# NVlabs/FB-BEV

Hardware: AMD Instinct MI355X
Metric: multi-cam samples/sec (forward view transformation: lift + voxel ranking + bev_pool_v2) (higher is better)
Workload: dtype f32

## Files before the change

fb_bev_amd/csrc/capi.hip:

```cpp
#include <stdio.h>
#include <stdlib.h>
#include <mutex>
#include "rt.h"
#include "pool_kernels.h"
#include "pool_bwd_kernels.h"
#include "rank_kernels.h"
#include "sort_kernels.h"
#include "msda_kernels.h"
#include "geom_kernels.h"
#include "da_kernels.h"
#include "history_kernels.h"
#include "norm_kernels.h"
#include "history_conv_kernels.h"
#include "history_fused_kernels.h"
#include "history_conv_x3_kernels.h"
#include "history_fused_x3_kernels.h"
#include "rows_linear_kernels.h"
#include "rows_linear_f32_kernels.h"
#include "da_fused_kernels.h"
#include "da_bwd_planes_kernels.h"
#include "msda_bwd_kernels.h"
#include "conv3d_kernels.h"
#include "det_kernels.h"
#include "occ_kernels.h"
#include "../../include/fbbev.h"

#include "capi_common.h"

extern "C" int fbbev_version(void) { return 100; }

extern "C" int fbbev_bev_pool_v2_fwd(int c, int n_intervals, const float* depth, const float* feat,
                                     const int32_t* ranks_depth, const int32_t* ranks_feat,
                                     const int32_t* ranks_bev, const int32_t* interval_starts,
                                     const int32_t* interval_lengths, float* out,
                                     fbbev_stream_t stream_) {
    if (c <= 0 || n_intervals < 0) return FBBEV_E_BADARG;
    if (n_intervals == 0) return 0;
    if (!depth || !feat || !ranks_depth || !ranks_feat || !ranks_bev || !interval_starts ||
        !interval_lengths || !out) return FBBEV_E_BADARG;
    fbbev_rt_stream stream = (fbbev_rt_stream)stream_;
    if (c % 4 == 0 && aligned16(feat) && aligned16(out)) {
        const long long threads = (long long)n_intervals * (c / 4);
        FBBEV_LAUNCH(k_pool_fwd_rows<4>, (threads + 255) / 256, 256, 0, stream, c, n_intervals, depth,
                     feat, ranks_depth, ranks_feat, ranks_bev, interval_starts, interval_lengths, out);
    } else {
        const long long threads = (long long)n_intervals * c;
        FBBEV_LAUNCH(k_pool_fwd_rows<1>, (threads + 255) / 256, 256, 0, stream, c, n_intervals, depth,
                     feat, ranks_depth, ranks_feat, ranks_bev, interval_starts, interval_lengths, out);
    }
    FBBEV_CHECK_LAUNCH();
    return 0;
}

extern "C" int fbbev_bev_pool_v2_bwd(int c, int n_intervals, const float* out_grad,
                                     const float* depth, const float* feat,
                                     const int32_t* ranks_depth, const int32_t* ranks_feat,
                                     const int32_t* ranks_bev, const int32_t* interval_starts,
                                     const int32_t* interval_lengths, float* depth_grad,
                                     float* feat_grad, fbbev_stream_t stream_) {
    if (c <= 0 || n_intervals < 0) return FBBEV_E_BADARG;
    if (c > 256) return FBBEV_E_UNSUPPORTED;
    if (n_intervals == 0) return 0;
    if (!out_grad || !depth || !feat || !ranks_depth || !ranks_feat || !ranks_bev ||
        !interval_starts || !interval_lengths || !depth_grad || !feat_grad) return FBBEV_E_BADARG;
    fbbev_rt_stream stream = (fbbev_rt_stream)stream_;
    const long long blocks = ((long long)n_intervals * 64 + 255) / 256;
    const int nch = (c + 63) / 64;
#define FBBEV_BWD(NCH)                                                                             \
    FBBEV_LAUNCH(k_pool_bwd<NCH>, blocks, 256, 0, stream, c, n_intervals, out_grad, depth, feat,   \
                 ranks_depth, ranks_feat, ranks_bev, interval_starts, interval_lengths, depth_grad, \
                 feat_grad)
    switch (nch) {
        case 1: FBBEV_BWD(1); break;
        case 2: FBBEV_BWD(2); break;
        case 3: FBBEV_BWD(3); break;
        default: FBBEV_BWD(4); break;
    }
#undef FBBEV_BWD
    FBBEV_CHECK_LAUNCH();
    return 0;
}

extern "C" int fbbev_lidar_coor(const float* xs, const float* ys, const float* ds, const float* rots,
                                const float* trans, const float* intrins, const float* post_rots,
                                const float* post_trans, const float* bda, int B, int N, int D, int H,
                                int W, float* coor, fbbev_stream_t stream_) {
    if (B <= 0 || N <= 0 || D <= 0 || H <= 0 || W <= 0) return FBBEV_E_BADARG;
    if (!xs || !ys || !ds || !rots || !trans || !intrins || !post_rots || !post_trans || !bda || !coor)
        return FBBEV_E_BADARG;
    const long long dhw = (long long)D * H * W;
    const long long chunks = (dhw + 255) / 256;
    if (chunks * B * N >= (1ll << 31)) return FBBEV_E_UNSUPPORTED;
    fbbev_cam_ptrs g;
    g.xs = xs; g.ys = ys; g.ds = ds; g.rots = rots; g.trans = trans; g.intrins = intrins; g.post_rots = post_rots;
    g.post_trans = post_trans; g.bda = bda; g.N = N; g.D = D; g.H = H; g.W = W;
    FBBEV_LAUNCH(k_lidar_coor, chunks * B * N, 256, 0, (fbbev_rt_stream)stream_, g, (int)chunks, coor);
    FBBEV_CHECK_LAUNCH();
    return 0;
}

extern "C" int fbbev_nchw_to_nhwc(const float* in, float* out, int n_images, int C, int HW, fbbev_stream_t stream_) {
    return fbbev_tokens_from_nchw(in, out, n_images, C, HW, (long long)C * HW, 0, nullptr, 0, stream_);
}

static int tokens_from_nchw_impl(const float* in, float* out, int n_images, int C, int HW, long long out_image_stride,
                                 long long out_offset, const float* bias, int bias_rows, const float* pos_bias,
                                 fbbev_stream_t stream_) {
    if (n_images < 0 || C <= 0 || HW <= 0 || out_offset < 0 || out_image_stride < (long long)C * HW) return FBBEV_E_BADARG;
    if (bias && bias_rows <= 0) return FBBEV_E_BADARG;
    if (n_images == 0) return 0;
    if (!in || !out) return FBBEV_E_BADARG;
    const int tc = (C + 31) / 32, th = (HW + 31) / 32;
    const long long blocks = (long long)n_images * tc * th;
    if (blocks >= (1ll << 31)) return FBBEV_E_UNSUPPORTED;
    FBBEV_LAUNCH(k_nchw_to_nhwc, blocks, 256, 0, (fbbev_rt_stream)stream_, in, out, C, HW, tc, th, out_image_stride,
                 out_offset, bias, bias ? bias_rows : 1, pos_bias);
    FBBEV_CHECK_LAUNCH();
    return 0;
}

extern "C" int fbbev_tokens_from_nchw(const float* in, float* out, int n_images, int C, int HW,
                                      long long out_image_stride, long long out_offset, const float* bias,
                                      int bias_rows, fbbev_stream_t stream_) {
    return tokens_from_nchw_impl(in, out, n_images, C, HW, out_image_stride, out_offset, bias, bias_rows, nullptr, stream_);
}

extern "C" int fbbev_tokens_from_nchw_levels(const float* const* in, const int32_t* hw, int n_levels, float* out, int n_images, int C,
                                             const float* bias, int bias_rows, fbbev_stream_t stream_) {
    if (n_levels <= 0 || n_levels > 8 || n_images < 0 || C <= 0 || !in || !hw) return FBBEV_E_BADARG;
    if (bias && bias_rows <= 0) return FBBEV_E_BADARG;
    if (n_images == 0) return 0;
    if (!out) return FBBEV_E_BADARG;
    fbbev_token_levels lv;
    const int tc = (C + 31) / 32;
    long long start = 0, blocks = 0;
    for (int l = 0; l < 8; ++l) { lv.in[l] = nullptr; lv.out_off[l] = 0; lv.hw[l] = 1; lv.blk0[l] = 0; }
    for (int l = 0; l < n_levels; ++l) {
        if (hw[l] <= 0 || !in[l]) return FBBEV_E_BADARG;
        lv.in[l] = in[l]; lv.hw[l] = hw[l]; lv.out_off[l] = start * C; lv.blk0[l] = (int)blocks;
        start += hw[l];
        blocks += (long long)n_images * tc * ((hw[l] + 31) / 32);
        if (blocks >= (1ll << 31)) return FBBEV_E_UNSUPPORTED;
    }
    lv.blk0[n_levels] = (int)blocks;
    lv.n = n_levels;
    FBBEV_LAUNCH(k_nchw_to_nhwc_levels, blocks, 256, 0, (fbbev_rt_stream)stream_, lv, out, C, tc, start * C, bias, bias ? bias_rows : 1);
    FBBEV_CHECK_LAUNCH();
    return 0;
}

extern "C" int fbbev_tokens_from_nchw_pos(const float* in, float* out, int n_images, int C, int HW, long long out_image_stride,
                                          long long out_offset, const float* pos_bias, fbbev_stream_t stream_) {
    if (!pos_bias) return FBBEV_E_BADARG;
    return tokens_from_nchw_impl(in, out, n_images, C, HW, out_image_stride, out_offset, nullptr, 0, pos_bias, stream_);
}

extern "C" int fbbev_point_sampling(const float* xs, const float* ys, const float* zs, const float* rots,
                                    const float* trans, const float* intrins, const float* post_rots,
                                    const float* post_trans, const float* bda, int B, int N, int Y, int X,
                                    int Za, float ogfH, float ogfW, float* ref_cam, uint8_t* mask,
                                    float* qdepth, fbbev_stream_t stream_) {
    if (B <= 0 || N <= 0 || Y <= 0 || X <= 0 || Za <= 0 || !(ogfH > 0.f) || !(ogfW > 0.f)) return FBBEV_E_BADARG;
    if (!xs || !ys || !zs || !rots || !trans || !intrins || !post_rots || !post_trans || !bda || !ref_cam ||
        !mask || !qdepth) return FBBEV_E_BADARG;
    const long long npts = (long long)Y * X * Za;
    int ppt = 8;
    while (ppt > 1 && (npts + 256 * ppt - 1) / (256 * ppt) * B * N < 1024) ppt >>= 1;
    const long long chunks = (npts + 256 * ppt - 1) / (256 * ppt);
    if (chunks * B * N >= (1ll << 31) || ((uintptr_t)ref_cam & 7) != 0) return FBBEV_E_UNSUPPORTED;
    FBBEV_LAUNCH(k_point_sampling, chunks * B * N, 256, 0, (fbbev_rt_stream)stream_, xs, ys, zs, rots, trans,
                 intrins, post_rots, post_trans, bda, B, N, Y, X, Za, ogfH, ogfW, (int)chunks, ref_cam, mask,
                 qdepth, ppt);
    FBBEV_CHECK_LAUNCH();
    return 0;
}

static inline int key_bits(long long total_voxels) {
    int bits = 1;
    while ((1ll << bits) < total_voxels) ++bits;
    return bits;
}

static const int kSortTile[7] = {2048, 4096, 8192, 12288, 16384, 4096, 8192};
static int sort_variant_for(long long items) {
    for (int v = 0; v < 5; ++v)
        if ((items + kSortTile[v] - 1) / kSortTile[v] <= 256) return v;
    return 6;
}
static const int kIvTile[3] = {1024, 4096, 8192};
static int iv_variant_for(long long items) {
    for (int v = 0; v < 3; ++v)
        if ((items + kIvTile[v] - 1) / kIvTile[v] <= 256) return v;
    return 2;
}

static fbbev_fastdiv make_fastdiv(unsigned int d) {
    fbbev_fastdiv f;
    f.d = d; f.m = 0; f.sh = 0;
    if (d <= 1) { f.d = 1; return f; }
    unsigned int l = 0;
    while ((1ull << l) < d) ++l;
    f.m = (unsigned int)((((1ull << l) - d) << 32) / d + 1);
    f.sh = l - 1;
    return f;
}

struct rank_ws_layout {
    size_t keys_a, keys_t, vals_t, matrix, ctot, chunk_info, total;
    int v0, wgs0;
    int v1, wgs1;
    int vi, wgsi;
};

static rank_ws_layout rank_layout(long long n) {
    rank_ws_layout L;
    L.v0 = sort_variant_for(n);
    L.v1 = sort_variant_for((n + 1) / 2);
    L.vi = iv_variant_for((n + 1) / 2);
    if (const char* env = fbbev_env_str("FBBEV_RANK_SHAPE")) {
        int a = -1, b = -1, c = -1;
        if (sscanf(env, "%d,%d,%d", &a, &b, &c) == 3 && a >= 0 && a < 7 && b >= 0 && b < 7 && c >= 0 && c < 3) {
            L.v0 = a; L.v1 = b; L.vi = c;
        }
    }
    L.wgs0 = (int)((n + kSortTile[L.v0] - 1) / kSortTile[L.v0]);
    L.wgs1 = (int)((n + kSortTile[L.v1] - 1) / kSortTile[L.v1]);
    L.wgsi = (int)((n + kIvTile[L.vi] - 1) / kIvTile[L.vi]);
    size_t off = 0;
    L.keys_a = off; off = align_up(off + (size_t)n * 4, 256);
    L.keys_t = off; off = align_up(off + (size_t)n * 4, 256);
    L.vals_t = off; off = align_up(off + (size_t)n * 4, 256);
    const int rows = L.wgs0 > L.wgs1 ? L.wgs0 : L.wgs1;
    const size_t seg_rows = (size_t)(n / FBBEV_SEG_TILE) + 256 + 1;
    size_t mbytes = (size_t)rows * FBBEV_SORT_MAX_NB * 4;
    if (seg_rows * FBBEV_SEG_NB * 4 > mbytes) mbytes = seg_rows * FBBEV_SEG_NB * 4;
    L.matrix = off; off = align_up(off + mbytes, 256);
    L.ctot = off; off = align_up(off + seg_rows * 4, 256);
    L.chunk_info = off; off = align_up(off + (size_t)L.wgsi * 8, 256);
    L.total = off;
    return L;
}

#define FBBEV_SORT_DISPATCH(KERNEL, v, by_waves, grid, stream, ...)                                             \
    do {                                                                                                        \
        switch (v) {                                                                                            \
            case 0: FBBEV_LAUNCH((KERNEL<(by_waves) ? 4 : 256, 8>), grid, 256, 0, stream, __VA_ARGS__); break;   \
            case 1: FBBEV_LAUNCH((KERNEL<(by_waves) ? 16 : 1024, 4>), grid, 1024, 0, stream, __VA_ARGS__); break; \
            case 2: FBBEV_LAUNCH((KERNEL<(by_waves) ? 16 : 1024, 8>), grid, 1024, 0, stream, __VA_ARGS__); break; \
            case 3: FBBEV_LAUNCH((KERNEL<(by_waves) ? 16 : 1024, 12>), grid, 1024, 0, stream, __VA_ARGS__); break; \
            case 5: FBBEV_LAUNCH((KERNEL<(by_waves) ? 8 : 512, 8>), grid, 512, 0, stream, __VA_ARGS__); break;     \
            case 6: FBBEV_LAUNCH((KERNEL<(by_waves) ? 8 : 512, 16>), grid, 512, 0, stream, __VA_ARGS__); break;    \
            default: FBBEV_LAUNCH((KERNEL<(by_waves) ? 16 : 1024, 16>), grid, 1024, 0, stream, __VA_ARGS__); break; \
        }                                                                                                       \
    } while (0)

extern "C" size_t fbbev_rank_workspace_bytes(int64_t n_points) {
    if (n_points <= 0) return 256;
    return rank_layout(n_points).total;
}

static int rank_seg_mode() { FBBEV_KNOB_ONCE(int, m, fbbev_env_int("FBBEV_RANK_SEG", -1)); return m; }

static int rank_build_impl(const float* coor, const fbbev_cam_ptrs* cams, const float* frustum, int B, int N, int D,
                           int H, int W,
                           const float* lower3, const float* interval3, const float* grid_size3,
                           int32_t* ranks_bev, int32_t* ranks_depth, int32_t* ranks_feat,
                           int32_t* interval_starts, int32_t* interval_lengths, int32_t* interval_rank,
                           int32_t* counts, void* workspace, size_t workspace_bytes, fbbev_rt_stream stream,
                           const float* point_depth = nullptr, float depth_thr = 0.f, const int* skip = nullptr) {
    if (B <= 0 || N <= 0 || D <= 0 || H <= 0 || W <= 0) return FBBEV_E_BADARG;
    if (point_depth && cams) return FBBEV_E_UNSUPPORTED;
    if ((!coor && !cams) || !lower3 || !interval3 || !grid_size3 || !ranks_bev || !ranks_depth || !ranks_feat ||
        !interval_starts || !interval_lengths || !counts || !workspace) return FBBEV_E_BADARG;
    const long long n = (long long)B * N * D * H * W;
    if (n >= (1ll << 30)) return FBBEV_E_UNSUPPORTED;
    const rank_ws_layout L = rank_layout(n);
    if (workspace_bytes < L.total) return FBBEV_E_WORKSPACE;
    unsigned char* ws = static_cast<unsigned char*>(workspace);
    unsigned int* keys_a = reinterpret_cast<unsigned int*>(ws + L.keys_a);
    unsigned int* keys_t = reinterpret_cast<unsigned int*>(ws + L.keys_t);
    unsigned int* vals_t = reinterpret_cast<unsigned int*>(ws + L.vals_t);
    int* matrix = reinterpret_cast<int*>(ws + L.matrix);
    int2* chunk_info = reinterpret_cast<int2*>(ws + L.chunk_info);

    fbbev_grid_params gp;
    gp.lx = lower3[0]; gp.ly = lower3[1]; gp.lz = lower3[2];
    gp.ix = interval3[0]; gp.iy = interval3[1]; gp.iz = interval3[2];
    gp.gx = grid_size3[0]; gp.gy = grid_size3[1]; gp.gz = grid_size3[2];
    volatile float zy = gp.gz * gp.gy;
    volatile float zyx = zy * gp.gx;
    volatile float yx = gp.gy * gp.gx;
    gp.f_zyx = zyx; gp.f_yx = yx;
    const long long total_voxels = (long long)B * (long long)gp.gz * (long long)gp.gy * (long long)gp.gx;
    if (total_voxels <= 0 || total_voxels >= (1ll << 30)) return FBBEV_E_UNSUPPORTED;
    const int bits = key_bits(total_voxels + 128);
    struct { int passes, rb; } plan;
    plan.passes = (bits + FBBEV_SORT_MAX_RB - 1) / FBBEV_SORT_MAX_RB;
    plan.rb = (bits + plan.passes - 1) / plan.passes;
    if (plan.rb < 4) plan.rb = 4;
    const int rb = plan.rb;
    const int seg_mode = rank_seg_mode();
    const long long vps = total_voxels / B;
    const long long npb = n / B;
    const int lbits = key_bits(vps);
    const bool seg_legal = B <= 256 && total_voxels <= (1ll << 24) && lbits <= 2 * FBBEV_SEG_RB;
    const long long seg_cps = (npb + FBBEV_SEG_TILE - 1) / FBBEV_SEG_TILE;
    const bool seg = seg_legal && seg_mode != 0 &&
                     (seg_mode == 2 || ((lbits + FBBEV_SEG_RB - 1) / FBBEV_SEG_RB < plan.passes && seg_cps <= 64 && B * seg_cps >= 96));
    if (seg) {
        fbbev_seg sg;
        sg.npb = (int)npb; sg.cps = (int)((npb + FBBEV_SEG_TILE - 1) / FBBEV_SEG_TILE); sg.vps = (unsigned int)vps; sg.nseg = B;
        const int passes = (lbits + FBBEV_SEG_RB - 1) / FBBEV_SEG_RB;
        const int srb = (lbits + passes - 1) / passes < 4 ? 4 : (lbits + passes - 1) / passes;
        const int wgs = B * sg.cps;
        int* ctot = reinterpret_cast<int*>(ws + L.ctot);
        fbbev_geom_src gs;
        if (cams) { gs.cam = *cams; gs.frustum = frustum; gs.gp = gp; }
        else { gs.cam = fbbev_cam_ptrs(); gs.frustum = nullptr; gs.gp = gp; }
        if (cams) FBBEV_LAUNCH((k_keys_hist_seg<true>), wgs, FBBEV_SEG_NT, 0, stream, gs, (const float*)nullptr, gp, (const float*)nullptr, 0.f,
                               sg, srb, skip, keys_a, matrix, ctot);
        else FBBEV_LAUNCH((k_keys_hist_seg<false>), wgs, FBBEV_SEG_NT, 0, stream, gs, coor, gp, point_depth, depth_thr, sg, srb, skip, keys_a,
                          matrix, ctot);
        FBBEV_CHECK_LAUNCH();
        const unsigned int* kin = keys_a;
        const unsigned int* vin = nullptr;
        static const int pairs = fbbev_env_int("FBBEV_RANK_PAIRS", 1);
        for (int p = 0; p < passes; ++p) {
            const bool to_out = p == passes - 1;
            const int pm = pairs ? ((p > 0 ? 1 : 0) | (to_out ? 0 : 2)) : 0;
            unsigned int* ko = to_out ? reinterpret_cast<unsigned int*>(ranks_bev) : keys_t;
            unsigned int* vo = to_out ? reinterpret_cast<unsigned int*>(ranks_depth) : vals_t;
            if (p > 0) {
                FBBEV_LAUNCH(k_sort_hist_seg, wgs, FBBEV_SEG_NT, 0, stream, kin, (const int*)ctot, sg, p * srb, srb, skip, matrix,
                             (pm & 1) ? 2 : 1);
                FBBEV_CHECK_LAUNCH();
            }
            static const int swz = fbbev_env_int("FBBEV_RANK_XCD_SWIZZLE", 1);
            const int sw = (swz && B >= 8) ? 1 : 0;
            FBBEV_LAUNCH(k_sort_scatter_seg, sw ? (wgs + 7) / 8 * 8 : wgs, FBBEV_SEG_NT, 0, stream, kin, vin, (const int*)matrix,
                         (const int*)ctot, sg, p, srb, skip, ko, vo, counts, sw, pm);
            FBBEV_CHECK_LAUNCH();
            kin = ko; vin = vo;
        }
    } else {
    if (cams) {
            fbbev_geom_src gs;
            gs.cam = *cams; gs.frustum = frustum; gs.gp = gp;
            FBBEV_SORT_DISPATCH(k_keys_hist_geom, L.v0, false, L.wgs0, stream, gs, n, rb, skip, keys_a, matrix);
        } else {
            FBBEV_SORT_DISPATCH(k_keys_hist_coor, L.v0, false, L.wgs0, stream, coor, n, n / B, gp, point_depth, depth_thr, rb, keys_a, matrix);
        }
        FBBEV_CHECK_LAUNCH();
        const unsigned int* kin = keys_a;
        const unsigned int* vin = nullptr;
        for (int p = 0; p < plan.passes; ++p) {
            const bool to_out = ((plan.passes - 1 - p) % 2) == 0;
            unsigned int* ko = to_out ? reinterpret_cast<unsigned int*>(ranks_bev) : keys_t;
            unsigned int* vo = to_out ? reinterpret_cast<unsigned int*>(ranks_depth) : vals_t;
            const int v = p == 0 ? L.v0 : L.v1, wgs = p == 0 ? L.wgs0 : L.wgs1;
            if (p > 0) {
                FBBEV_SORT_DISPATCH(k_sort_hist, v, false, wgs, stream, kin, (const int*)counts, p * rb, rb, skip, matrix);
                FBBEV_CHECK_LAUNCH();
            }
            static const int swz = fbbev_env_int("FBBEV_RANK_XCD_SWIZZLE", 1);
            const bool sw = swz == 2 && p == 0;
            FBBEV_SORT_DISPATCH(k_sort_scatter, v, true, sw ? (wgs + 7) / 8 * 8 : wgs, stream, kin, vin, n, (const int*)matrix, p, rb, skip,
                                ko, vo, counts, sw ? wgs : 0);
            FBBEV_CHECK_LAUNCH();
            kin = ko; vin = vo;
        }
}
    const unsigned int* keys = reinterpret_cast<const unsigned int*>(ranks_bev);
    const unsigned int* vals = reinterpret_cast<const unsigned int*>(ranks_depth);
    const fbbev_fastdiv div_dhw = make_fastdiv((unsigned int)((long long)D * H * W)), div_hw = make_fastdiv((unsigned int)(H * W));
    switch (L.vi) {
        case 0:
            FBBEV_LAUNCH((k_interval_count<4, 4>), L.wgsi, 256, 0, stream, keys, (const int*)counts, skip, chunk_info);
            FBBEV_LAUNCH((k_interval_write<4, 4>), L.wgsi, 256, (size_t)2 * 4 * 256 * 4, stream, keys, vals, div_dhw, div_hw, (const int2*)chunk_info, skip,
                         ranks_feat, interval_starts, interval_lengths, interval_rank, counts);
            break;
        case 1:
            FBBEV_LAUNCH((k_interval_count<16, 4>), L.wgsi, 1024, 0, stream, keys, (const int*)counts, skip, chunk_info);
            FBBEV_LAUNCH((k_interval_write<16, 4>), L.wgsi, 1024, (size_t)2 * 4 * 1024 * 4, stream, keys, vals, div_dhw, div_hw, (const int2*)chunk_info, skip,
                         ranks_feat, interval_starts, interval_lengths, interval_rank, counts);
            break;
        default:
            FBBEV_LAUNCH((k_interval_count<16, 8>), L.wgsi, 1024, 0, stream, keys, (const int*)counts, skip, chunk_info);
            FBBEV_LAUNCH((k_interval_write<16, 8>), L.wgsi, 1024, (size_t)2 * 8 * 1024 * 4, stream, keys, vals, div_dhw, div_hw, (const int2*)chunk_info, skip,
                         ranks_feat, interval_starts, interval_lengths, interval_rank, counts);
            break;
    }
    FBBEV_CHECK_LAUNCH();
    return 0;
}

extern "C" int fbbev_rank_build(const float* coor, int B, int N, int D, int H, int W,
                                const float* lower3, const float* interval3,
                                const float* grid_size3, int32_t* ranks_bev, int32_t* ranks_depth,
                                int32_t* ranks_feat, int32_t* interval_starts,
                                int32_t* interval_lengths, int32_t* interval_rank, int32_t* counts,
                                void* workspace, size_t workspace_bytes, fbbev_stream_t stream_) {
    if (!coor) return FBBEV_E_BADARG;
    return rank_build_impl(coor, nullptr, nullptr, B, N, D, H, W, lower3, interval3, grid_size3, ranks_bev, ranks_depth,
                           ranks_feat, interval_starts, interval_lengths, interval_rank, counts, workspace,
                           workspace_bytes, (fbbev_rt_stream)stream_);
}

extern "C" int fbbev_rank_build_depth(const float* coor, const float* depth, float depth_threshold, int B, int N, int D,
                                      int H, int W, const float* lower3, const float* interval3,
                                      const float* grid_size3, int32_t* ranks_bev, int32_t* ranks_depth,
                                      int32_t* ranks_feat, int32_t* interval_starts, int32_t* interval_lengths,
                                      int32_t* interval_rank, int32_t* counts, void* workspace, size_t workspace_bytes,
                                      fbbev_stream_t stream_) {
    if (!coor || !depth) return FBBEV_E_BADARG;
    return rank_build_impl(coor, nullptr, nullptr, B, N, D, H, W, lower3, interval3, grid_size3, ranks_bev, ranks_depth,
                           ranks_feat, interval_starts, interval_lengths, interval_rank, counts, workspace,
                           workspace_bytes, (fbbev_rt_stream)stream_, depth, depth_threshold);
}

static int lift_rank_build_impl(const float* frustum, const float* xs, const float* ys, const float* ds,
                                const float* rots, const float* trans, const float* intrins, const float* post_rots,
                                const float* post_trans, const float* bda, int B, int N, int D, int H, int W,
                                const float* lower3, const float* interval3, const float* grid_size3,
                                int32_t* ranks_bev, int32_t* ranks_depth, int32_t* ranks_feat, int32_t* interval_starts,
                                int32_t* interval_lengths, int32_t* interval_rank, int32_t* counts, void* workspace,
                                size_t workspace_bytes, fbbev_rt_stream stream, uint32_t* cam_key, int32_t* cache_state) {
    if (!xs || !ys || !ds || !rots || !trans || !intrins || !post_rots || !post_trans || !bda) return FBBEV_E_BADARG;
    if (B <= 0 || N <= 0) return FBBEV_E_BADARG;
    fbbev_cam_ptrs g;
    g.xs = xs; g.ys = ys; g.ds = ds; g.rots = rots; g.trans = trans; g.intrins = intrins; g.post_rots = post_rots;
    g.post_trans = post_trans; g.bda = bda; g.N = N; g.D = D; g.H = H; g.W = W;
    const int* skip = nullptr;
    if (cam_key) {
        if (!cache_state) return FBBEV_E_BADARG;
        FBBEV_LAUNCH(k_cam_key, 1, 256, 0, stream, g, B, cam_key, cache_state);
        FBBEV_CHECK_LAUNCH();
        skip = cache_state;
    }
    return rank_build_impl(nullptr, &g, frustum, B, N, D, H, W, lower3, interval3, grid_size3, ranks_bev, ranks_depth,
                           ranks_feat, interval_starts, interval_lengths, interval_rank, counts, workspace,
                           workspace_bytes, stream, nullptr, 0.f, skip);
}

extern "C" int fbbev_lift_rank_build(const float* frustum, const float* xs, const float* ys, const float* ds,
                                     const float* rots,
                                     const float* trans, const float* intrins, const float* post_rots,
                                     const float* post_trans, const float* bda, int B, int N, int D, int H,
                                     int W, const float* lower3, const float* interval3,
                                     const float* grid_size3, int32_t* ranks_bev, int32_t* ranks_depth,
                                     int32_t* ranks_feat, int32_t* interval_starts, int32_t* interval_lengths,
                                     int32_t* interval_rank, int32_t* counts, void* workspace,
                                     size_t workspace_bytes, fbbev_stream_t stream_) {
    return lift_rank_build_impl(frustum, xs, ys, ds, rots, trans, intrins, post_rots, post_trans, bda, B, N, D, H, W, lower3,
                                interval3, grid_size3, ranks_bev, ranks_depth, ranks_feat, interval_starts,
                                interval_lengths, interval_rank, counts, workspace, workspace_bytes,
                                (fbbev_rt_stream)stream_, nullptr, nullptr);
}

extern "C" size_t fbbev_cam_key_words(int B, int N) {
    return (B <= 0 || N <= 0) ? 0 : (size_t)B * N * 33 + (size_t)B * 9;
}

extern "C" int fbbev_lift_rank_build_cached(const float* frustum, const float* xs, const float* ys, const float* ds,
                                            const float* rots, const float* trans, const float* intrins,
                                            const float* post_rots, const float* post_trans, const float* bda, int B,
                                            int N, int D, int H, int W, const float* lower3, const float* interval3,
                                            const float* grid_size3, int32_t* ranks_bev, int32_t* ranks_depth,
                                            int32_t* ranks_feat, int32_t* interval_starts, int32_t* interval_lengths,
                                            int32_t* interval_rank, int32_t* counts, void* workspace,
                                            size_t workspace_bytes, uint32_t* cam_key, int32_t* cache_state,
                                            fbbev_stream_t stream_) {
    if (!cam_key || !cache_state) return FBBEV_E_BADARG;
    return lift_rank_build_impl(frustum, xs, ys, ds, rots, trans, intrins, post_rots, post_trans, bda, B, N, D, H, W, lower3,
                                interval3, grid_size3, ranks_bev, ranks_depth, ranks_feat, interval_starts,
                                interval_lengths, interval_rank, counts, workspace, workspace_bytes,
                                (fbbev_rt_stream)stream_, cam_key, cache_state);
}

static inline int pick_tile(int tile_voxels) {
    switch (tile_voxels) { case 64: case 128: case 256: case 512: case 1024: return tile_voxels; default: return 64; }
}
static inline int small_tile_shift(int tile_voxels) {
    switch (tile_voxels) { case 8: return 3; case 16: return 4; case 32: return 5; default: return 0; }
}

extern "C" size_t fbbev_pool_dense_workspace_bytes(int B, int Z, int Y, int X) {
    if (B <= 0 || Z <= 0 || Y <= 0 || X <= 0) return 256;
    const long long yx = (long long)Y * X;
    const long long tiles = ((long long)B * Z * yx + 7) / 8 + (long long)B * Z;
    return align_up((size_t)(tiles + 2) * 8, 256);
}

static int pool_tile_index_impl(const int32_t* interval_rank, const int32_t* interval_starts,
// ... 3173 lines not shown
```

fb_bev_amd/csrc/sort_kernels.h:

```cpp
#pragma once
#include "rt.h"
#include "geom_kernels.h"
#include "rank_kernels.h"

#define FBBEV_SORT_MAX_RB 8
#define FBBEV_SORT_MAX_NB (1 << FBBEV_SORT_MAX_RB)
#define FBBEV_SORT_MAX_PASSES 4
#define FBBEV_DROP_KEY 0xffffffffu

__device__ __forceinline__ bool fbbev_skip(const int* skip) { return skip != nullptr && *skip != 0; }

struct fbbev_geom_src {
    fbbev_cam_ptrs cam;
    const float* frustum;
    fbbev_grid_params gp;
};

__device__ __forceinline__ unsigned int fbbev_geom_key(const fbbev_geom_src& g, const float* m, int cam, int i) {
    float u, v, dep;
    if (g.frustum) {
        u = g.frustum[3 * i]; v = g.frustum[3 * i + 1]; dep = g.frustum[3 * i + 2];
    } else {
        const int w = i % g.cam.W, h = (i / g.cam.W) % g.cam.H, d = i / (g.cam.W * g.cam.H);
        u = g.cam.xs[w]; v = g.cam.ys[h]; dep = g.cam.ds[d];
// ... 67 lines not shown
            if (key != FBBEV_DROP_KEY) atomicAdd(&cnt[key & dmask], 1);
        }
    }
    __syncthreads();
    for (int d = threadIdx.x; d < nb; d += NT) matrix[(long long)blockIdx.x * nb + d] = cnt[d];
}

template <int NT, int PER>
__global__ void __launch_bounds__(NT)
k_sort_hist(const unsigned int* __restrict__ keys, const int* __restrict__ counts, int shift, int rb,
            const int* __restrict__ skip, int* __restrict__ matrix) {
    if (fbbev_skip(skip)) return;
    __shared__ int cnt[FBBEV_SORT_MAX_NB];
    const int nb = 1 << rb;
    const unsigned int dmask = (unsigned int)nb - 1u;
    const long long n = counts[0];
    const long long base = (long long)blockIdx.x * (NT * PER);
    if (base >= n) return;
    for (int d = threadIdx.x; d < nb; d += NT) cnt[d] = 0;
    __syncthreads();
    unsigned int key[PER];
#pragma unroll
    for (int r = 0; r < PER; ++r) {
        const long long idx = base + threadIdx.x + r * NT;
        key[r] = (idx < n) ? keys[idx] : FBBEV_DROP_KEY;
    }
#pragma unroll
    for (int r = 0; r < PER; ++r)
        if (key[r] != FBBEV_DROP_KEY) atomicAdd(&cnt[(key[r] >> shift) & dmask], 1);
    __syncthreads();
    for (int d = threadIdx.x; d < nb; d += NT) matrix[(long long)blockIdx.x * nb + d] = cnt[d];
}

template <int WAVES, int ROUNDS>
__global__ void __launch_bounds__(WAVES * 64)
k_sort_scatter(const unsigned int* __restrict__ keys_in, const unsigned int* __restrict__ vals_in, long long n_host,
               const int* __restrict__ matrix, int pass, int rb, const int* __restrict__ skip,
               unsigned int* __restrict__ keys_out, unsigned int* __restrict__ vals_out, int* __restrict__ counts, int swz_chunks) {
    if (fbbev_skip(skip)) return;
    constexpr int NT = WAVES * 64;
    constexpr int TILE = NT * ROUNDS;
    constexpr int NBM = FBBEV_SORT_MAX_NB;
    __shared__ int cnt[WAVES][NBM];
    __shared__ int woff[WAVES][NBM];
    __shared__ int pos0[NBM];
    __shared__ int ldsw[WAVES];
    const int tid = threadIdx.x, wave = tid >> 6, lane = tid & 63;
    const int nb = 1 << rb, shift = pass * rb;
    const unsigned int dmask = (unsigned int)nb - 1u;
    int wg = (int)blockIdx.x;
    if (swz_chunks > 0) {
        wg = (int)(blockIdx.x & 7) * ((swz_chunks + 7) >> 3) + (int)(blockIdx.x >> 3);
        if (wg >= swz_chunks) return;
    }
    const long long n = (pass == 0) ? n_host : (long long)counts[0];
    const long long chunk0 = (long long)wg * TILE;
    if (chunk0 >= n) {
        if (pass == 0 && n_host <= 0 && wg == 0 && tid == 0) counts[0] = 0;
        return;
    }
    for (int i = tid; i < WAVES * NBM; i += NT) (&cnt[0][0])[i] = 0;
    const int rows = (int)((n + TILE - 1) / TILE);
    {
        const int groups = NT / nb > 0 ? NT / nb : 1;
        int pre = 0, all = 0;
        if (tid < groups * nb) {
            const int d = tid % nb, rg = tid / nb;
            constexpr int U = 8;
            int r = rg;
            for (; r + (U - 1) * groups < rows; r += U * groups) {
                int c[U];
#pragma unroll
                for (int u = 0; u < U; ++u) c[u] = matrix[(long long)(r + u * groups) * nb + d];
#pragma unroll
                for (int u = 0; u < U; ++u) { all += c[u]; if (r + u * groups < wg) pre += c[u]; }
            }
            for (; r < rows; r += groups) {
                const int c = matrix[(long long)r * nb + d];
                all += c;
                if (r < wg) pre += c;
            }
        }
        int* red = &woff[0][0];
        __syncthreads();
        if (tid < groups * nb) { red[tid] = pre; red[groups * nb + tid] = all; }
        __syncthreads();
        int mypre = 0, myall = 0;
        if (tid < nb) {
            for (int gi = 0; gi < groups; ++gi) { mypre += red[gi * nb + tid]; myall += red[groups * nb + gi * nb + tid]; }
        }
        __syncthreads();
        int total;
        const int dbase = fbbev_block_excl_scan_w<WAVES, false>(tid < nb ? myall : 0, ldsw, &total);
        if (tid < nb) pos0[tid] = dbase + mypre;
        if (pass == 0 && wg == 0 && tid == 0) counts[0] = total;
    }
    const long long chunk = chunk0 + (long long)wave * (64 * ROUNDS);
    unsigned int k[ROUNDS], v[ROUNDS];
    int lr[ROUNDS];
    const unsigned long long lt = (lane == 0) ? 0ull : (~0ull >> (64 - lane));
#pragma unroll
    for (int r = 0; r < ROUNDS; ++r) {
        const long long idx = chunk + r * 64 + lane;
        const bool valid = idx < n;
        k[r] = valid ? keys_in[idx] : FBBEV_DROP_KEY;
        v[r] = valid ? (vals_in ? vals_in[idx] : (unsigned int)idx) : 0u;
    }
#pragma unroll
    for (int r = 0; r < ROUNDS; ++r) {
        const bool valid = k[r] != FBBEV_DROP_KEY;
        lr[r] = -1;
        const unsigned int d = (k[r] >> shift) & dmask;
        unsigned long long mm = __ballot(valid ? 1 : 0);
#pragma unroll
        for (int bit = 0; bit < FBBEV_SORT_MAX_RB; ++bit) {
            if (bit < rb) {
                const unsigned long long b = __ballot((int)((d >> bit) & 1u));
                mm &= ((d >> bit) & 1u) ? b : ~b;
            }
        }
        const int leader = valid ? (__ffsll((long long)mm) - 1) : lane;
        int prev = 0;
        if (valid && lane == leader) {
            prev = cnt[wave][d];
            cnt[wave][d] = prev + __popcll(mm);
        }
        prev = __shfl(prev, leader, 64);
        if (valid) lr[r] = prev + __popcll(mm & lt);
    }
    __syncthreads();
    for (int d = tid; d < nb; d += NT) {
        int run = pos0[d];
#pragma unroll
        for (int w = 0; w < WAVES; ++w) { woff[w][d] = run; run += cnt[w][d]; }
    }
    __syncthreads();
#pragma unroll
    for (int r = 0; r < ROUNDS; ++r) {
        if (lr[r] >= 0) {
            const unsigned int d = (k[r] >> shift) & dmask;
            const int pos = woff[wave][d] + lr[r];
            keys_out[pos] = k[r];
            vals_out[pos] = v[r];
        }
    }
}

#define FBBEV_SEG_RB 10
#define FBBEV_SEG_NB (1 << FBBEV_SEG_RB)
#define FBBEV_SEG_WAVES 8
#define FBBEV_SEG_ROUNDS 16
#define FBBEV_SEG_NT (FBBEV_SEG_WAVES * 64)
#define FBBEV_SEG_TILE (FBBEV_SEG_NT * FBBEV_SEG_ROUNDS)

struct fbbev_seg {
    int npb;
    int cps;
    unsigned int vps;
    int nseg;
};

template <int WAVES>
__device__ __forceinline__ void fbbev_seg_prefix2(const int* __restrict__ ctot, int lo, int hi, int* red, int& sum_lo, int& sum_hi) {
    int a = 0, b = 0;
    for (int i = threadIdx.x; i < hi; i += WAVES * 64) {
        const int c = ctot[i];
        b += c;
        if (i < lo) a += c;
    }
#pragma unroll
    for (int o = 32; o > 0; o >>= 1) { a += __shfl_down(a, o, 64); b += __shfl_down(b, o, 64); }
    const int wave = threadIdx.x >> 6;
    if ((threadIdx.x & 63) == 0) { red[2 * wave] = a; red[2 * wave + 1] = b; }
    __syncthreads();
    sum_lo = 0; sum_hi = 0;
#pragma unroll
    for (int w = 0; w < WAVES; ++w) { sum_lo += red[2 * w]; sum_hi += red[2 * w + 1]; }
    __syncthreads();
}

template <bool GEOM>
__global__ void __launch_bounds__(FBBEV_SEG_NT)
k_keys_hist_seg(fbbev_geom_src g, const float* __restrict__ coor, fbbev_grid_params gp, const float* __restrict__ depth,
                float depth_thr, fbbev_seg sg, int rb, const int* __restrict__ skip, unsigned int* __restrict__ keys_out,
                int* __restrict__ matrix, int* __restrict__ ctot) {
    if (fbbev_skip(skip)) return;
    constexpr int NT = FBBEV_SEG_NT, PER = FBBEV_SEG_ROUNDS;
    __shared__ int cnt[FBBEV_SEG_NB];
    __shared__ float m[33];
    __shared__ int tot;
    const int nb = 1 << rb;
    const unsigned int dmask = (unsigned int)nb - 1u;
    for (int d = threadIdx.x; d < nb; d += NT) cnt[d] = 0;
    if (threadIdx.x == 0) tot = 0;
    const int b = blockIdx.x / sg.cps, c = blockIdx.x - b * sg.cps;
    const int base = b * sg.npb + c * FBBEV_SEG_TILE;
    const int lim = (b + 1) * sg.npb;
    const int end = base + FBBEV_SEG_TILE < lim ? base + FBBEV_SEG_TILE : lim;
    const unsigned int kbase = (unsigned int)b * sg.vps;
    int mine = 0;
    if constexpr (GEOM) {
        const int dhw = g.cam.D * g.cam.H * g.cam.W;
        const int cam_lo = base / dhw, cam_hi = (end > base ? end - 1 : base) / dhw;
        constexpr int G = 8;
        for (int cam = cam_lo; cam <= cam_hi; ++cam) {
            __syncthreads();
            if (threadIdx.x == 0) fbbev_cam_setup(g.cam, cam, m);
            __syncthreads();
            const int c0 = cam * dhw;
            const int lo = base > c0 ? base : c0, hi = end < c0 + dhw ? end : c0 + dhw;
            for (int r0 = 0; r0 < PER; r0 += G) {
                unsigned int key[G];
#pragma unroll
                for (int r = 0; r < G; ++r) {
                    const int pid = base + (int)threadIdx.x + (r0 + r) * NT;
                    key[r] = (pid >= lo && pid < hi) ? fbbev_geom_key(g, m, cam, pid - c0) : FBBEV_DROP_KEY;
                }
#pragma unroll
                for (int r = 0; r < G; ++r) {
                    const int pid = base + (int)threadIdx.x + (r0 + r) * NT;
                    if (pid >= lo && pid < hi) {
                        keys_out[pid] = key[r];
                        if (key[r] != FBBEV_DROP_KEY) { atomicAdd(&cnt[(key[r] - kbase) & dmask], 1); ++mine; }
                    }
                }
            }
        }
    } else {
        __syncthreads();
#pragma unroll
        for (int r = 0; r < PER; ++r) {
            const int pid = base + (int)threadIdx.x + r * NT;
            if (pid < end) {
                unsigned int key = fbbev_rank_key(coor[3 * (long long)pid], coor[3 * (long long)pid + 1], coor[3 * (long long)pid + 2], gp,
                                                  (float)b, FBBEV_DROP_KEY);
                if (depth && !(depth[pid] > depth_thr)) key = FBBEV_DROP_KEY;
                keys_out[pid] = key;
                if (key != FBBEV_DROP_KEY) { atomicAdd(&cnt[(key - kbase) & dmask], 1); ++mine; }
            }
        }
    }
#pragma unroll
    for (int o = 32; o > 0; o >>= 1) mine += __shfl_down(mine, o, 64);
    if ((threadIdx.x & 63) == 0 && mine) atomicAdd(&tot, mine);
    __syncthreads();
    for (int d = threadIdx.x; d < nb; d += NT) matrix[(long long)blockIdx.x * nb + d] = cnt[d];
    if (threadIdx.x == 0) ctot[blockIdx.x] = tot;
}

__global__ void __launch_bounds__(FBBEV_SEG_NT)
k_sort_hist_seg(const unsigned int* __restrict__ keys, const int* __restrict__ ctot, fbbev_seg sg, int shift, int rb,
                const int* __restrict__ skip, int* __restrict__ matrix, int key_stride) {
    if (fbbev_skip(skip)) return;
    constexpr int NT = FBBEV_SEG_NT, PER = FBBEV_SEG_ROUNDS;
    __shared__ int cnt[FBBEV_SEG_NB];
    __shared__ int red[2 * FBBEV_SEG_WAVES];
    const int nb = 1 << rb;
    const unsigned int dmask = (unsigned int)nb - 1u;
    const int b = blockIdx.x / sg.cps, c = blockIdx.x - b * sg.cps;
    for (int d = threadIdx.x; d < nb; d += NT) cnt[d] = 0;
    int s0, s1;
    fbbev_seg_prefix2<FBBEV_SEG_WAVES>(ctot, b * sg.cps, (b + 1) * sg.cps, red, s0, s1);
    const long long base = (long long)s0 + (long long)c * FBBEV_SEG_TILE;
    const unsigned int kbase = (unsigned int)b * sg.vps;
    if (base < s1) {
        unsigned int key[PER];
#pragma unroll
        for (int r = 0; r < PER; ++r) {
            const long long idx = base + threadIdx.x + r * NT;
            key[r] = (idx < s1) ? keys[idx * key_stride] : FBBEV_DROP_KEY;
        }
#pragma unroll
        for (int r = 0; r < PER; ++r)
            if (key[r] != FBBEV_DROP_KEY) atomicAdd(&cnt[((key[r] - kbase) >> shift) & dmask], 1);
    }
    __syncthreads();
    for (int d = threadIdx.x; d < nb; d += NT) matrix[(long long)blockIdx.x * nb + d] = cnt[d];
}

__global__ void __launch_bounds__(FBBEV_SEG_NT)
k_sort_scatter_seg(const unsigned int* __restrict__ keys_in, const unsigned int* __restrict__ vals_in, const int* __restrict__ matrix,
                   const int* __restrict__ ctot, fbbev_seg sg, int pass, int rb, const int* __restrict__ skip,
                   unsigned int* __restrict__ keys_out, unsigned int* __restrict__ vals_out, int* __restrict__ counts, int xcd_swizzle, int pair_mode) {
    if (fbbev_skip(skip)) return;
    constexpr int WAVES = FBBEV_SEG_WAVES, ROUNDS = FBBEV_SEG_ROUNDS, NT = FBBEV_SEG_NT, NBM = FBBEV_SEG_NB;
    int chunk_id = (int)blockIdx.x;
    if (xcd_swizzle) {
        const int total = sg.nseg * sg.cps, per_xcd = (total + 7) >> 3;
        chunk_id = (int)(blockIdx.x & 7) * per_xcd + (int)(blockIdx.x >> 3);
        if (chunk_id >= total) return;
    }
    __shared__ __attribute__((aligned(16))) int cnt[WAVES][NBM];
    __shared__ int pos0[NBM];
    __shared__ int red[2 * WAVES];
    __shared__ int ldsw[WAVES];
    const int tid = threadIdx.x, wave = tid >> 6, lane = tid & 63;
    const int nb = 1 << rb, shift = pass * rb;
    const unsigned int dmask = (unsigned int)nb - 1u;
    const int b = chunk_id / sg.cps, c = chunk_id - b * sg.cps;
    const unsigned int kbase = (unsigned int)b * sg.vps;
    int s0, s1;
    fbbev_seg_prefix2<WAVES>(ctot, b * sg.cps, (b + 1) * sg.cps, red, s0, s1);
    if (pass == 0 && chunk_id == 0) {
        int p0, pall;
        fbbev_seg_prefix2<WAVES>(ctot, 0, sg.nseg * sg.cps, red, p0, pall);
        if (tid == 0) counts[0] = pall;
    }
    const long long in0 = pass == 0 ? (long long)b * sg.npb : (long long)s0;
    const long long in1 = pass == 0 ? (long long)(b + 1) * sg.npb : (long long)s1;
    const long long chunk0 = in0 + (long long)c * FBBEV_SEG_TILE;
    if (chunk0 >= in1) return;
    const long long chunk = chunk0 + (long long)wave * (64 * ROUNDS);
    unsigned int k[ROUNDS], v[ROUNDS];
    int lr[ROUNDS];
    const unsigned long long lt = (lane == 0) ? 0ull : (~0ull >> (64 - lane));
#pragma unroll
    for (int r = 0; r < ROUNDS; ++r) {
        const long long idx = chunk + r * 64 + lane;
        const bool valid = idx < in1;
        if (pair_mode & 1) {
            uint2 kv = make_uint2(FBBEV_DROP_KEY, 0u);
            if (valid) kv = reinterpret_cast<const uint2*>(keys_in)[idx];
            k[r] = kv.x; v[r] = kv.y;
        } else {
            k[r] = valid ? keys_in[idx] : FBBEV_DROP_KEY;
            v[r] = valid ? (vals_in ? vals_in[idx] : (unsigned int)idx) : 0u;
        }
    }
    const int row0 = b * sg.cps;
    {
        const int nq = nb >> 2;
        const int quad = tid % nq, rg = tid / nq;
        fbbev_v4i pre = {0, 0, 0, 0}, all = {0, 0, 0, 0};
        if (rg < 2) {
            constexpr int U = 8;
            const int* col = matrix + (long long)row0 * nb + 4 * quad;
            for (int r = rg; r < sg.cps; r += 2 * U) {
                fbbev_v4i t[U];
#pragma unroll
                for (int u = 0; u < U; ++u) {
                    const int rr = r + 2 * u < sg.cps ? r + 2 * u : sg.cps - 1;
                    __builtin_memcpy(&t[u], col + (long long)rr * nb, 16);
                }
#pragma unroll
                for (int u = 0; u < U; ++u) {
                    if (r + 2 * u < sg.cps) all += t[u];
                    if (r + 2 * u < c) pre += t[u];
                }
            }
            __builtin_memcpy(&cnt[1 + rg][4 * quad], &pre, 16);
            __builtin_memcpy(&cnt[3 + rg][4 * quad], &all, 16);
        }
    }
    __syncthreads();
    {
        const int d0 = 2 * tid, d1 = 2 * tid + 1;
        const int a0 = d0 < nb ? cnt[3][d0] + cnt[4][d0] : 0, a1 = d1 < nb ? cnt[3][d1] + cnt[4][d1] : 0;
        const int p0 = d0 < nb ? cnt[1][d0] + cnt[2][d0] : 0, p1 = d1 < nb ? cnt[1][d1] + cnt[2][d1] : 0;
        int total;
        const int ex = fbbev_block_excl_scan_w<WAVES, false>(a0 + a1, ldsw, &total);
        if (d0 < nb) pos0[d0] = p0 + s0 + ex;
        if (d1 < nb) pos0[d1] = p1 + s0 + ex + a0;
    }
    __syncthreads();
    for (int i = tid; i < WAVES * NBM; i += NT) (&cnt[0][0])[i] = 0;
    __syncthreads();
#pragma unroll
    for (int r = 0; r < ROUNDS; ++r) {
        const bool valid = k[r] != FBBEV_DROP_KEY;
        lr[r] = -1;
        const unsigned int d = ((k[r] - kbase) >> shift) & dmask;
        unsigned long long mm = __ballot(valid ? 1 : 0);
#pragma unroll
        for (int bit = 0; bit < FBBEV_SEG_RB; ++bit) {
            if (bit < rb) {
                const unsigned long long bb = __ballot((int)((d >> bit) & 1u));
                mm &= ((d >> bit) & 1u) ? bb : ~bb;
            }
        }
        const int leader = valid ? (__ffsll((long long)mm) - 1) : lane;
        int prev = 0;
        if (valid && lane == leader) {
            prev = cnt[wave][d];
            cnt[wave][d] = prev + __popcll(mm);
        }
        prev = __shfl(prev, leader, 64);
        if (valid) lr[r] = prev + __popcll(mm & lt);
    }
    __syncthreads();
    for (int d = tid; d < nb; d += NT) {
        int run = pos0[d];
#pragma unroll
        for (int w = 0; w < WAVES; ++w) { const int t = cnt[w][d]; cnt[w][d] = run; run += t; }
    }
    __syncthreads();
#pragma unroll
    for (int r = 0; r < ROUNDS; ++r) {
        if (lr[r] >= 0) {
            const unsigned int d = ((k[r] - kbase) >> shift) & dmask;
            const int pos = cnt[wave][d] + lr[r];
            if (pair_mode & 2) reinterpret_cast<uint2*>(keys_out)[pos] = make_uint2(k[r], v[r]);
            else { keys_out[pos] = k[r]; vals_out[pos] = v[r]; }
        }
    }
}

__global__ void __launch_bounds__(256)
k_cam_key(fbbev_cam_ptrs g, int B, unsigned int* __restrict__ key, int* __restrict__ state) {
    __shared__ int differ;
    if (threadIdx.x == 0) differ = 0;
    __syncthreads();
    const int cams = B * g.N;
    const float* src[6] = {g.rots, g.trans, g.intrins, g.post_rots, g.post_trans, g.bda};
    const int len[6] = {cams * 9, cams * 3, cams * 9, cams * 9, cams * 3, B * 9};
    int off = 0, bad = 0;
    for (int s = 0; s < 6; ++s) {
        for (int i = threadIdx.x; i < len[s]; i += 256) {
            unsigned int bits;
            const float f = src[s][i];
            __builtin_memcpy(&bits, &f, 4);
            bad |= (bits != key[off + i]) ? 1 : 0;
        }
        off += len[s];
    }
    if (bad) differ = 1;
    __syncthreads();
    if (!differ) { if (threadIdx.x == 0) state[0] = 1; return; }
    off = 0;
    for (int s = 0; s < 6; ++s) {
        for (int i = threadIdx.x; i < len[s]; i += 256) {
            unsigned int bits;
            const float f = src[s][i];
            __builtin_memcpy(&bits, &f, 4);
            key[off + i] = bits;
        }
        off += len[s];
    }
    if (threadIdx.x == 0) { state[0] = 0; state[1] += 1; }
}
```

Baseline: 23010.

## Use LDS bitmask table for wave digit matching and optionally fold pass-1 histogram

Replaces the per-bit ballot loop used for warp-level digit matching in the segmented radix scatter with an LDS table of 64-bit lane masks. Lanes atomically OR their bit into a per-wave slot indexed by the low digit bits, and ballots are kept only for the remaining high bits. Optionally, the second-pass histogram is accumulated with global atomics during the first scatter, which removes the separate histogram kernel, but that path is off by default. This adds LDS use and extra wave syncs per round in exchange for fewer ballot instructions.

```diff
diff --git a/fb_bev_amd/csrc/capi.hip b/fb_bev_amd/csrc/capi.hip
--- a/fb_bev_amd/csrc/capi.hip
+++ b/fb_bev_amd/csrc/capi.hip
@@ -1,5 +1,6 @@
 #include <stdio.h>
 #include <stdlib.h>
+#include <string.h>
 #include <mutex>
 #include "rt.h"
 #include "pool_kernels.h"
@@ -206,7 +207,7 @@
 }
 
 struct rank_ws_layout {
-    size_t keys_a, keys_t, vals_t, matrix, ctot, chunk_info, total;
+    size_t keys_a, keys_t, vals_t, matrix, matrix1, ctot, chunk_info, total;
     int v0, wgs0;
     int v1, wgs1;
     int vi, wgsi;
@@ -235,6 +236,7 @@
     size_t mbytes = (size_t)rows * FBBEV_SORT_MAX_NB * 4;
     if (seg_rows * FBBEV_SEG_NB * 4 > mbytes) mbytes = seg_rows * FBBEV_SEG_NB * 4;
     L.matrix = off; off = align_up(off + mbytes, 256);
+    L.matrix1 = off; off = align_up(off + seg_rows * FBBEV_SEG_NB * 4, 256);
     L.ctot = off; off = align_up(off + seg_rows * 4, 256);
     L.chunk_info = off; off = align_up(off + (size_t)L.wgsi * 8, 256);
     L.total = off;
@@ -260,6 +262,21 @@
 }
 
 static int rank_seg_mode() { FBBEV_KNOB_ONCE(int, m, fbbev_env_int("FBBEV_RANK_SEG", -1)); return m; }
+#define FBBEV_RANK_MATCH_DEFAULT 9
+static int rank_match_parse(const char* e) {
+    if (e && !strcmp(e, "ballot")) return 0;
+    if (e && !strcmp(e, "table8")) return 8;
+    if (e && !strcmp(e, "table9")) return 9;
+    return FBBEV_RANK_MATCH_DEFAULT;
+}
+static int rank_match_bits() { FBBEV_KNOB_ONCE(int, t, rank_match_parse(fbbev_env_str("FBBEV_RANK_MATCH"))); return t; }
+#define FBBEV_RANK_HIST1_DEFAULT 0
+static int rank_hist1_parse(const char* e) {
+    if (e && !strcmp(e, "kernel")) return 0;
+    if (e && !strcmp(e, "pass0")) return 1;
+    return FBBEV_RANK_HIST1_DEFAULT;
+}
+static bool rank_hist1_folded() { FBBEV_KNOB_ONCE(int, f, rank_hist1_parse(fbbev_env_str("FBBEV_RANK_HIST1"))); return f != 0; }
 
 static int rank_build_impl(const float* coor, const fbbev_cam_ptrs* cams, const float* frustum, int B, int N, int D,
                            int H, int W,
@@ -314,13 +331,15 @@
         const int srb = (lbits + passes - 1) / passes < 4 ? 4 : (lbits + passes - 1) / passes;
         const int wgs = B * sg.cps;
         int* ctot = reinterpret_cast<int*>(ws + L.ctot);
+        int* matrix1 = (passes == 2 && rank_hist1_folded()) ? reinterpret_cast<int*>(ws + L.matrix1) : nullptr;
+        const int tbits = rank_match_bits() == 0 ? 0 : (srb < rank_match_bits() ? srb : rank_match_bits());
         fbbev_geom_src gs;
         if (cams) { gs.cam = *cams; gs.frustum = frustum; gs.gp = gp; }
         else { gs.cam = fbbev_cam_ptrs(); gs.frustum = nullptr; gs.gp = gp; }
         if (cams) FBBEV_LAUNCH((k_keys_hist_seg<true>), wgs, FBBEV_SEG_NT, 0, stream, gs, (const float*)nullptr, gp, (const float*)nullptr, 0.f,
-                               sg, srb, skip, keys_a, matrix, ctot);
+                               sg, srb, skip, keys_a, matrix, ctot, matrix1);
         else FBBEV_LAUNCH((k_keys_hist_seg<false>), wgs, FBBEV_SEG_NT, 0, stream, gs, coor, gp, point_depth, depth_thr, sg, srb, skip, keys_a,
-                          matrix, ctot);
+                          matrix, ctot, matrix1);
         FBBEV_CHECK_LAUNCH();
         const unsigned int* kin = keys_a;
         const unsigned int* vin = nullptr;
@@ -330,15 +349,16 @@
             const int pm = pairs ? ((p > 0 ? 1 : 0) | (to_out ? 0 : 2)) : 0;
             unsigned int* ko = to_out ? reinterpret_cast<unsigned int*>(ranks_bev) : keys_t;
             unsigned int* vo = to_out ? reinterpret_cast<unsigned int*>(ranks_depth) : vals_t;
-            if (p > 0) {
+            if (p > 0 && !matrix1) {
                 FBBEV_LAUNCH(k_sort_hist_seg, wgs, FBBEV_SEG_NT, 0, stream, kin, (const int*)ctot, sg, p * srb, srb, skip, matrix,
                              (pm & 1) ? 2 : 1);
                 FBBEV_CHECK_LAUNCH();
             }
             static const int swz = fbbev_env_int("FBBEV_RANK_XCD_SWIZZLE", 1);
             const int sw = (swz && B >= 8) ? 1 : 0;
-            FBBEV_LAUNCH(k_sort_scatter_seg, sw ? (wgs + 7) / 8 * 8 : wgs, FBBEV_SEG_NT, 0, stream, kin, vin, (const int*)matrix,
-                         (const int*)ctot, sg, p, srb, skip, ko, vo, counts, sw, pm);
+            FBBEV_LAUNCH(k_sort_scatter_seg, sw ? (wgs + 7) / 8 * 8 : wgs, FBBEV_SEG_NT, 0, stream, kin, vin,
+                         (const int*)((p > 0 && matrix1) ? matrix1 : matrix), (const int*)ctot, sg, p, srb, skip, ko, vo, counts, sw, pm,
+                         tbits, p == 0 ? matrix1 : (int*)nullptr);
             FBBEV_CHECK_LAUNCH();
             kin = ko; vin = vo;
         }
diff --git a/fb_bev_amd/csrc/sort_kernels.h b/fb_bev_amd/csrc/sort_kernels.h
--- a/fb_bev_amd/csrc/sort_kernels.h
+++ b/fb_bev_amd/csrc/sort_kernels.h
@@ -243,6 +243,25 @@
 #define FBBEV_SEG_ROUNDS 16
 #define FBBEV_SEG_NT (FBBEV_SEG_WAVES * 64)
 #define FBBEV_SEG_TILE (FBBEV_SEG_NT * FBBEV_SEG_ROUNDS)
+#define FBBEV_SEG_TMIN 8
+#define FBBEV_SEG_TMAX 9
+#ifdef FBBEV_TEST_OVERRIDES
+inline void fbbev_lds_or_u64(unsigned long long* p, unsigned long long v) { *p |= v; }
+inline unsigned long long fbbev_lds_ld_u64(const unsigned long long* p) { return *p; }
+inline void fbbev_lds_st_u64(unsigned long long* p, unsigned long long v) { *p = v; }
+inline void fbbev_lds_wait() {}
+#else
+__device__ __forceinline__ void fbbev_lds_wait() { __builtin_amdgcn_s_waitcnt(0xc07f); }
+__device__ __forceinline__ void fbbev_lds_or_u64(unsigned long long* p, unsigned long long v) {
+    (void)__hip_atomic_fetch_or(p, v, __ATOMIC_RELAXED, __HIP_MEMORY_SCOPE_WORKGROUP);
+}
+__device__ __forceinline__ unsigned long long fbbev_lds_ld_u64(const unsigned long long* p) {
+    return __hip_atomic_load(p, __ATOMIC_RELAXED, __HIP_MEMORY_SCOPE_WORKGROUP);
+}
+__device__ __forceinline__ void fbbev_lds_st_u64(unsigned long long* p, unsigned long long v) {
+    __hip_atomic_store(p, v, __ATOMIC_RELAXED, __HIP_MEMORY_SCOPE_WORKGROUP);
+}
+#endif
 
 struct fbbev_seg {
     int npb;
@@ -274,7 +293,7 @@
 __global__ void __launch_bounds__(FBBEV_SEG_NT)
 k_keys_hist_seg(fbbev_geom_src g, const float* __restrict__ coor, fbbev_grid_params gp, const float* __restrict__ depth,
                 float depth_thr, fbbev_seg sg, int rb, const int* __restrict__ skip, unsigned int* __restrict__ keys_out,
-                int* __restrict__ matrix, int* __restrict__ ctot) {
+                int* __restrict__ matrix, int* __restrict__ ctot, int* __restrict__ matrix1) {
     if (fbbev_skip(skip)) return;
     constexpr int NT = FBBEV_SEG_NT, PER = FBBEV_SEG_ROUNDS;
     __shared__ int cnt[FBBEV_SEG_NB];
@@ -283,6 +302,7 @@
     const int nb = 1 << rb;
     const unsigned int dmask = (unsigned int)nb - 1u;
     for (int d = threadIdx.x; d < nb; d += NT) cnt[d] = 0;
+    if (matrix1) for (int d = threadIdx.x; d < nb; d += NT) matrix1[(long long)blockIdx.x * nb + d] = 0;
     if (threadIdx.x == 0) tot = 0;
     const int b = blockIdx.x / sg.cps, c = blockIdx.x - b * sg.cps;
     const int base = b * sg.npb + c * FBBEV_SEG_TILE;
@@ -372,7 +392,8 @@
 __global__ void __launch_bounds__(FBBEV_SEG_NT)
 k_sort_scatter_seg(const unsigned int* __restrict__ keys_in, const unsigned int* __restrict__ vals_in, const int* __restrict__ matrix,
                    const int* __restrict__ ctot, fbbev_seg sg, int pass, int rb, const int* __restrict__ skip,
-                   unsigned int* __restrict__ keys_out, unsigned int* __restrict__ vals_out, int* __restrict__ counts, int xcd_swizzle, int pair_mode) {
+                   unsigned int* __restrict__ keys_out, unsigned int* __restrict__ vals_out, int* __restrict__ counts, int xcd_swizzle, int pair_mode,
+                   int tbits, int* __restrict__ matrix1) {
     if (fbbev_skip(skip)) return;
     constexpr int WAVES = FBBEV_SEG_WAVES, ROUNDS = FBBEV_SEG_ROUNDS, NT = FBBEV_SEG_NT, NBM = FBBEV_SEG_NB;
     int chunk_id = (int)blockIdx.x;
@@ -383,11 +404,13 @@
     }
     __shared__ __attribute__((aligned(16))) int cnt[WAVES][NBM];
     __shared__ int pos0[NBM];
+    __shared__ __attribute__((aligned(16))) unsigned long long tbl[WAVES][1 << FBBEV_SEG_TMAX];
     __shared__ int red[2 * WAVES];
     __shared__ int ldsw[WAVES];
     const int tid = threadIdx.x, wave = tid >> 6, lane = tid & 63;
     const int nb = 1 << rb, shift = pass * rb;
     const unsigned int dmask = (unsigned int)nb - 1u;
+    if (tbits > 0) for (int e = lane; e < (1 << tbits); e += 64) tbl[wave][e] = 0ull;
     const int b = chunk_id / sg.cps, c = chunk_id - b * sg.cps;
     const unsigned int kbase = (unsigned int)b * sg.vps;
     int s0, s1;
@@ -456,6 +479,48 @@
     __syncthreads();
     for (int i = tid; i < WAVES * NBM; i += NT) (&cnt[0][0])[i] = 0;
     __syncthreads();
+    if (tbits > 0) {
+        unsigned long long* tw = tbl[wave];
+        const unsigned int tmask = (1u << tbits) - 1u;
+        unsigned long long mm[ROUNDS];
+        fbbev_wave_sync();
+#pragma unroll
+        for (int r = 0; r < ROUNDS; ++r) {
+            const bool valid = k[r] != FBBEV_DROP_KEY;
+            const unsigned int e = ((k[r] - kbase) >> shift) & dmask & tmask;
+            if (valid) fbbev_lds_or_u64(&tw[e], 1ull << lane);
+            fbbev_wave_sync();
+            mm[r] = 0ull;
+            if (valid) mm[r] = fbbev_lds_ld_u64(&tw[e]);
+            fbbev_wave_sync();
+            if (valid) fbbev_lds_st_u64(&tw[e], 0ull);
+            fbbev_wave_sync();
+        }
+        fbbev_lds_wait();
+        int prev[ROUNDS], leader[ROUNDS];
+#pragma unroll
+        for (int r = 0; r < ROUNDS; ++r) {
+            const bool valid = k[r] != FBBEV_DROP_KEY;
+            const unsigned int d = ((k[r] - kbase) >> shift) & dmask;
+#pragma unroll
+            for (int bit = FBBEV_SEG_TMIN; bit < FBBEV_SEG_RB; ++bit) {
+                if (bit >= tbits && bit < rb) {
+                    const unsigned long long bb = __ballot((int)((d >> bit) & 1u));
+                    mm[r] &= ((d >> bit) & 1u) ? bb : ~bb;
+                }
+            }
+            leader[r] = valid ? (__ffsll((long long)mm[r]) - 1) : lane;
+            prev[r] = 0;
+            if (valid && lane == leader[r]) prev[r] = atomicAdd(&cnt[wave][d], __popcll(mm[r]));
+            lr[r] = valid ? __popcll(mm[r] & lt) : -1;
+            fbbev_wave_sync();
+        }
+#pragma unroll
+        for (int r = 0; r < ROUNDS; ++r) {
+            const int p = __shfl(prev[r], leader[r], 64);
+            if (lr[r] >= 0) lr[r] += p;
+        }
+    } else {
 #pragma unroll
     for (int r = 0; r < ROUNDS; ++r) {
         const bool valid = k[r] != FBBEV_DROP_KEY;
@@ -477,6 +542,7 @@
         }
         prev = __shfl(prev, leader, 64);
         if (valid) lr[r] = prev + __popcll(mm & lt);
+    }
     }
     __syncthreads();
     for (int d = tid; d < nb; d += NT) {
@@ -492,6 +558,7 @@
             const int pos = cnt[wave][d] + lr[r];
             if (pair_mode & 2) reinterpret_cast<uint2*>(keys_out)[pos] = make_uint2(k[r], v[r]);
             else { keys_out[pos] = k[r]; vals_out[pos] = v[r]; }
+            if (matrix1) atomicAdd(&matrix1[(long long)(row0 + (pos - s0) / FBBEV_SEG_TILE) * nb + (((k[r] - kbase) >> rb) & dmask)], 1);
         }
     }
 }
```

After: 23200, median of 6. No clear change (+0.8%).
